# ivargr/kmer_mapper

Measured on AMD Instinct MI355X. Metric: M k-mers mapped/sec (whole node), k=31 150bp reads, higher is better.
Workload: dtype u64

## Files before the change

### kmer_mapper_amd/csrc/kmm.hip

```cpp
#include <hip/hip_runtime.h>

#include <cstdarg>
#include <cstdint>
#include <cstdio>
#include <cstdlib>
#include <chrono>
#include <cstring>
#include <memory>
#include <mutex>
#include <string>
#include <thread>
#include <utility>
#include <vector>

#include "kmm.h"
#include "kmm_radix_plan.hpp"

namespace {

thread_local std::string g_err;

int fail(int code, const char *fmt, ...)
{
    char buf[1024];
// ... 287 lines not shown
    int64_t bgzf_carry_len = 0;
    BgzfStaged bgzf_pre;
    bool bgzf_pre_valid = false;
    const uint8_t *bgzf_pre_from = nullptr, *bgzf_hint_ptr = nullptr;
    int64_t bgzf_pre_n = 0, bgzf_hint_n = 0;
    int bgzf_pre_buf = 0;
    int64_t bgzf_prestaged_calls = 0;
    int64_t bgzf_head_skip = 0;
    int64_t bgzf_tail_stop = -1;
    int64_t bgzf_calls = 0, bgzf_members = 0;
    DevBuf gz_comp, gz_raw, gz_carry, gz_window, gz_tabs, gz_meta, gz_res, gz_win, gz_gmaps, gz_gwin, gz_err;
    std::vector<DevBuf> gz_arena;
    kmm_gunzip::StreamState gz_state;
    int64_t gz_carry_len = 0;
    double gz_ratio = 4.0;
    int64_t gzip_calls = 0, gzip_members = 0, gzip_chunks = 0, gzip_false_starts = 0, gzip_continuations = 0, gzip_inflated = 0;
    int dbg_gzip_chunk_kb = 0;
    DevBuf bam_tiles[2], bam_bad, bam_base, bam_ctl, bam_out;
    int32_t bam_n_ref = -1;
    uint32_t bam_excl = 0;
    int64_t bam_calls = 0, bam_records = 0, bam_excluded = 0, bam_header_bytes = 0, bam_false_starts = 0, bam_continuations = 0;
    int64_t dbg_bgzf_call_cap_kb = 0;
    int64_t flat_uniform_batches = 0;
    DevBuf sam_tiles, sam_base, sam_ctl;
    int64_t sam_calls = 0, sam_records = 0, sam_excluded = 0, sam_header_lines = 0;
    int dbg_bgzf_slot_kb = 0;
    int64_t dbg_rx_buf_limit = 0;
    int dbg_rec_copy_stream = 0;
    int dbg_rec_skip = 0;
    int min_base_quality = 0;
    int64_t dbg_rec_piece_kb = 0;
    bool rx_filter = true;
    bool rx_filter_slots = true;
    uint32_t dbg_p2f_cap = P2F_SLOTS;
    bool rx_packed = true;
    bool ecnt_dirty = false;
    bool rx_unchecked = false;
    DevBuf rx_buf1, rx_buf2, rx_meta, rx_probe;
    int sticky_rc = KMM_OK;
    std::string sticky_msg;
    uint64_t map_calls = 0;
    uint64_t n_radix_batches = 0, n_direct_batches = 0;
    ncclComm_t comm = nullptr;
    int comm_rank = -1, comm_size = 0;
    int comm_slices = 8;
    int64_t comm_sliced_reduces = 0;
    Stream comm_stream;
    std::vector<Event> comm_events;
    std::vector<uint64_t> flush_cuts;
    bool timing = false;
    std::vector<TimedEvent> ev_used;
    std::vector<TimedEvent> ev_free;
    double ms_total[KMM_N_KERNELS] = {0};
    int64_t launches[KMM_N_KERNELS] = {0};
};

namespace {

IndexView view_of(const kmm_index *ix)
{
    IndexView v;
    v.buckets = ix->buckets;
    v.entries = ix->entries;
    v.occ = ix->use_occ ? ix->occ : nullptr;
    v.occ_shift = ix->occ_shift;
    v.bloom_words = ix->bloom_words;
// ... 3135 lines not shown
{
    if (!ix || !name)
        return fail(KMM_ERR_INVALID_ARG, "NULL argument");
    HIPCHK(hipSetDevice(ix->device));
    if (strncmp(name, "debug_records_", 14) != 0)
        HIPCHK(hipStreamSynchronize(ix->stream));
    if (!strcmp(name, "path")) {
        if (value < 0 || value > 2)
            return fail(KMM_ERR_INVALID_ARG, "path must be 0 (auto), 1 (direct) or 2 (radix)");
        if (value == 2 && !ix->rx_ok)
            return fail(KMM_ERR_INVALID_ARG, "the radix path is not available for this index (modulo %llu: needs modulo < 2^31 "
                        "and slices whose entries fit LDS)", (unsigned long long)ix->modulo);
        ix->path = (int)value;
    } else if (!strcmp(name, "part_shift")) {
        const int rc = rx_reconfigure(ix, (int)value, -1, true);
        if (rc == RX_REFUSED)
            return fail(KMM_ERR_INVALID_ARG, "part_shift %lld: needs 0 <= shift <= 13, at most 512 x 512 fine partitions "
                        "and 2^shift small enough for the quotient of a 64-bit k-mer by the modulo to fit beside "
                        "the hash bits", (long long)value);
        KMMCHK(rc);
    } else if (!strcmp(name, "radix_packed_tiles")) {
        ix->rx_packed = value != 0;
    } else if (!strcmp(name, "radix_filter")) {
        ix->rx_filter = value != 0;
        if (ix->rx_pstart) {
            const int rc = rx_reconfigure(ix, ix->rx_geo.w, -1, false);
            if (rc != RX_REFUSED)
                KMMCHK(rc);
        }
    } else if (!strcmp(name, "radix_filter_slots")) {
        ix->rx_filter_slots = value != 0;
        if (ix->rx_pstart && ix->rx_ok)
            KMMCHK(rx_build_slots(ix));
    } else if (!strcmp(name, "debug_p2f_round_slots")) {
        if (value < 512 || value > P2F_SLOTS || (value & 1))
            return fail(KMM_ERR_INVALID_ARG, "debug_p2f_round_slots must be even and in [512, %d]", P2F_SLOTS);
        ix->dbg_p2f_cap = (uint32_t)value;
    } else if (!strcmp(name, "fine_bits")) {
        const int rc = value < 0 || value > 9 ? RX_REFUSED : rx_reconfigure(ix, ix->rx_geo.w, (int)value, true);
        if (rc == RX_REFUSED)
            return fail(KMM_ERR_INVALID_ARG, "fine_bits %lld: both fan-outs must stay within 512", (long long)value);
        KMMCHK(rc);
    } else if (!strcmp(name, "radix_min_units")) {
        ix->rx_min_units = value;
    } else if (!strcmp(name, "radix_sub_batch_kmers")) {
        if (value < 4 * RX_B || value > ((int64_t)1 << 32) - 2 * RX_B)
            return fail(KMM_ERR_INVALID_ARG, "radix_sub_batch_kmers outside [%d, 2^32 - %d]", 4 * RX_B, 2 * RX_B);
        ix->rx_sub_cap = value;
        ix->rx_sub_cap_eff = 0;
    } else if (!strcmp(name, "comm_overlap_slices")) {
        if (value < 1 || value > 64)
            return fail(KMM_ERR_INVALID_ARG, "comm_overlap_slices outside [1, 64]");
        ix->comm_slices = (int)value;
        ix->flush_cuts.clear();
    } else if (!strcmp(name, "radix_sorted_flush")) {
        ix->rx_flush_sorted = value != 0;
    } else if (!strcmp(name, "radix_grid_per_cu")) {
        if (value < 1 || value > 2)
            return fail(KMM_ERR_INVALID_ARG, "radix_grid_per_cu must be 1 or 2");
        ix->rx_grid_per_cu = (int)value;
    } else if (!strcmp(name, "count_kmers")) {
        if (value && !ix->rx_ok)
            return fail(KMM_ERR_INVALID_ARG, "count_kmers needs the radix path, which is not available for this index");
        KMMCHK(rx_flush(ix));
        HIPCHK(hipStreamSynchronize(ix->stream));
        if (value && !ix->rx_ecnt_acc) {
// ... 171 lines not shown
        } else {
            const size_t ld = (size_t)ix->dbg_F1 + 1;
            std::vector<uint16_t> r((size_t)ix->dbg_NB * ld);
            HIPCHK(hipMemcpy(r.data(), ix->dbg_start1, r.size() * 2, hipMemcpyDeviceToHost));
            for (size_t b = 0; b < ix->dbg_NB; ++b)
                sum += r[b * ld + ld - 1];
        }
        *value = (int64_t)sum;
    }
    else if (!strcmp(name, "radix_sorted_flush"))
        *value = (ix->rx_flush_sorted && ix->rx_norder) ? 1 : 0;
    else if (!strcmp(name, "radix_available"))
        *value = ix->rx_ok ? 1 : 0;
    else if (!strcmp(name, "radix_batches"))
        *value = (int64_t)ix->n_radix_batches;
    else if (!strcmp(name, "direct_batches"))
        *value = (int64_t)ix->n_direct_batches;
    else if (!strcmp(name, "radix_unavailable_reason"))
        *value = ix->rx_ok ? 0 : ix->rx_why_not;
    else if (!strcmp(name, "direct_view_resident"))
        *value = ix->buckets ? 1 : 0;
    else if (!strcmp(name, "direct_view_bytes"))
        *value = (int64_t)ix->direct_bytes;
    else if (!strcmp(name, "radix_view_bytes"))
        *value = ix->rx_pstart ? (int64_t)rx_view_bytes(ix->modulo, ix->rx_S, ix->rx_norder != nullptr) : 0;
    else if (!strcmp(name, "radix_filter"))
        *value = (ix->rx_ok && rx_filter_active(ix)) ? 1 : 0;
    else if (!strcmp(name, "radix_p3_keys_in_lds"))
        *value = ix->rx_ok ? rx_p3_shape(rx_p3_variant(ix)).keys_in_lds : 0;
    else if (!strcmp(name, "radix_filter_buckets_per_bit"))
        *value = (ix->rx_ok && rx_filter_active(ix)) ? (1 << ix->rx_geo.occ_shift) : 0;
    else if (!strcmp(name, "radix_filter_slots"))
        *value = (ix->rx_ok && rx_slots_active(ix)) ? 1 : 0;
    else if (!strcmp(name, "radix_filter_bits_per_partition"))
        *value = !(ix->rx_ok && rx_filter_active(ix)) ? 0
                 : rx_slots_active(ix)                ? (int64_t)P2F_SLOT_WORDS * 32
                                                      : (int64_t)1 << (ix->rx_geo.w + ix->rx_geo.f2 - ix->rx_geo.occ_shift);
    else if (!strcmp(name, "debug_p2f_round_slots"))
        *value = ix->dbg_p2f_cap;
    else if (!strcmp(name, "radix_packed_tiles"))
        *value = ix->rx_packed ? 1 : 0;
    else if (!strcmp(name, "n_fine_per_coarse"))
        *value = ix->rx_ok ? ix->rx_geo.F2 : 0;
    else if (!strcmp(name, "count_kmers"))
        *value = ix->rx_ecnt_acc ? 1 : 0;
    else if (!strcmp(name, "n_coarse_partitions"))
        *value = ix->rx_ok ? ix->rx_geo.F1 : 0;
    else if (!strcmp(name, "radix_p2_kmers") || !strcmp(name, "radix_p3_kmers") || !strcmp(name, "radix_p2_dropped") ||
             !strcmp(name, "radix_p2_multi_round_items") || !strcmp(name, "quality_masked_bases") || !strncmp(name, "stats_slot_", 11)) {
        HIPCHK(hipSetDevice(ix->device));
        KMMCHK(drain(ix));
        std::vector<unsigned long long> st(KMM_STAT_BYTES / 8);
        HIPCHK(hipMemcpy(st.data(), ix->stats, KMM_STAT_BYTES, hipMemcpyDeviceToHost));
        const int slot = name[0] == 's' ? atoi(name + 11) : name[0] == 'q' ? KMM_STAT_QUAL_MASKED
                                                          : !strcmp(name, "radix_p2_dropped") ? KMM_STAT_RX_DROPPED
                                                          : !strcmp(name, "radix_p2_multi_round_items") ? KMM_STAT_RX_MULTI
                                                          : name[7] == '2' ? 2 : 3;
        if (slot < 0 || slot >= KMM_STAT_STRIDE)
            return fail(KMM_ERR_INVALID_ARG, "unknown parameter '%s'", name);
        unsigned long long t = 0;
        for (int i = 0; i < KMM_STAT_SHARDS; ++i)
            t += st[(size_t)i * KMM_STAT_STRIDE + slot];
        *value = (int64_t)t;
    }
    else if (!strcmp(name, "grid_per_cu"))
        *value = ix->grid_per_cu;
    else if (!strcmp(name, "dynamic_schedule"))
        *value = ix->dynamic_schedule ? 1 : 0;
    else if (!strcmp(name, "occupancy_filter"))
        *value = (ix->use_occ && ix->occ) ? 1 : 0;
    else if (!strcmp(name, "bloom_filter_bytes"))
        *value = (ix->use_occ && ix->occ) ? (int64_t)ix->bloom_words * 4 : 0;
    else if (!strcmp(name, "occupancy_bits_per_bucket"))
        *value = (ix->use_occ && ix->occ && !ix->bloom_words) ? (1 << ix->occ_shift) : 0;
    else if (!strcmp(name, "wide_buckets"))
        *value = ix->wide ? 1 : 0;
    else if (!strcmp(name, "n_partitions"))
        *value = ix->rx_ok ? ix->rx_geo.PF : 0;
    else
        return fail(KMM_ERR_INVALID_ARG, "unknown parameter '%s'", name);
    return KMM_OK;
}

}
```

### kmer_mapper_amd/csrc/kmm_probe.hpp

```cpp
#pragma once

typedef uint32_t u32x4 __attribute__((ext_vector_type(4)));

struct IndexView {
    const uint4 *buckets;
    const uint4 *entries;
    const uint32_t *occ;
    int occ_shift;
    uint32_t bloom_words;
    int wide;
    uint32_t *counts;
    unsigned long long *stats;
    uint64_t modulo;
    uint64_t magic;
};

struct ReadsView {
    const uint8_t *bases;
    int64_t total;
    const int64_t *offsets;
    int64_t n_reads;
    const uint32_t *start_bits;
    int64_t n_start_words;
    uint64_t read_len;
// ... 43 lines not shown
    return q;
}


__device__ __forceinline__ uint32_t wave_scan_incl(uint32_t v)
{
    v += (uint32_t)__builtin_amdgcn_update_dpp(0, (int)v, 0x111, 0xF, 0xF, false);
    v += (uint32_t)__builtin_amdgcn_update_dpp(0, (int)v, 0x112, 0xF, 0xF, false);
    v += (uint32_t)__builtin_amdgcn_update_dpp(0, (int)v, 0x114, 0xF, 0xF, false);
    v += (uint32_t)__builtin_amdgcn_update_dpp(0, (int)v, 0x118, 0xF, 0xF, false);
    v += (uint32_t)__builtin_amdgcn_update_dpp(0, (int)v, 0x142, 0xA, 0xF, false);
    v += (uint32_t)__builtin_amdgcn_update_dpp(0, (int)v, 0x143, 0xC, 0xF, false);
    return v;
}

__device__ __forceinline__ uint64_t revcomp(uint64_t x, int k)
{
    x = ~x;
    x = ((x >> 2) & 0x3333333333333333ull) | ((x & 0x3333333333333333ull) << 2);
    x = ((x >> 4) & 0x0F0F0F0F0F0F0F0Full) | ((x & 0x0F0F0F0F0F0F0F0Full) << 4);
    x = ((x >> 8) & 0x00FF00FF00FF00FFull) | ((x & 0x00FF00FF00FF00FFull) << 8);
    x = ((x >> 16) & 0x0000FFFF0000FFFFull) | ((x & 0x0000FFFF0000FFFFull) << 16);
    x = (x >> 32) | (x << 32);
    return x >> (64 - 2 * k);
}

__device__ __forceinline__ uint32_t kmer_fp16(uint64_t q)
{
    return (uint32_t)((q * 0x9E3779B97F4A7C15ull) >> 48);
}

constexpr int KMM_STAT_SHARDS = 256;
constexpr int KMM_STAT_STRIDE = 32;
constexpr int KMM_STAT_RX_P1 = 16, KMM_STAT_RX_DROPPED = 17, KMM_STAT_RX_MULTI = 18, KMM_STAT_QUAL_MASKED = 19;
constexpr int AGG_LOG_SLOTS = 11;
constexpr int AGG_SLOTS = 1 << AGG_LOG_SLOTS;
constexpr uint32_t AGG_EMPTY = 0xFFFFFFFFu;

struct NodeAgg {
    uint32_t key[AGG_SLOTS];
    uint32_t val[AGG_SLOTS];
    uint32_t st[2];
};

__device__ __forceinline__ void agg_init(NodeAgg &agg)
{
    for (int i = threadIdx.x; i < AGG_SLOTS; i += blockDim.x) {
        agg.key[i] = AGG_EMPTY;
        agg.val[i] = 0;
    }
    if (threadIdx.x < 2)
        agg.st[threadIdx.x] = 0;
}

__device__ __forceinline__ void agg_add_n(const IndexView &iv, NodeAgg &agg, uint32_t node, uint32_t inc)
{
    const uint32_t slot = (node * 2654435761u) >> (32 - AGG_LOG_SLOTS);
    const uint32_t prev = atomicCAS(&agg.key[slot], AGG_EMPTY, node);
    if (prev == AGG_EMPTY || prev == node)
        atomicAdd(&agg.val[slot], inc);
    else
        atomicAdd(&iv.counts[node], inc);
}

__device__ __forceinline__ void agg_add(const IndexView &iv, NodeAgg &agg, uint32_t node, uint32_t &hits)
{
    ++hits;
// ... 208 lines not shown
```

### kmer_mapper_amd/csrc/kmm_radix.hpp

```cpp
#pragma once
#include <type_traits>
#include "kmm_radix_plan.hpp"

constexpr int RX_NT = 512;
constexpr int RX_KPT = RX_B / RX_NT;
#ifndef RX_LPR2V
#define RX_LPR2V 16
#endif
constexpr int RX_LPR = RX_LPR2V;
constexpr int RX_NG = RX_NT / RX_LPR;
#ifndef RX_RB1
#define RX_RB1 4
#endif
#ifndef RX_RB2
#define RX_RB2 8
#endif
constexpr int RX_SUBCAP = 1024;
#ifndef RX_SUBCAP3V
#define RX_SUBCAP3V 3072
#endif
constexpr int RX_SUBCAP3 = RX_SUBCAP3V;
#ifndef RX_LPR3
#define RX_LPR3 16
#endif
// ... 1356 lines not shown
        put_table(rd, item_lo(0), item_lo(0) + item_n(0), 0);
        if (n_it > 1u)
            rd = load_desc(s_b0[1]);
        __syncthreads();
        cover = t_vs[P2F_NT];
        vm0 = fill(std::false_type(), b0, item_lo(0), item_n(0), item_lo(0), cover, x0, 0);
        __syncthreads();
        if (cover < item_lo(0) + item_n(0))
            more_rounds(0, x0, vm0);
        if (tid < RX_B / 32)
            t_sbits[0][tid] = 0u;
        if (tid == 0)
            t_empty[0] = 0u;
        if (n_it > 1u) {
            put_table(rd, item_lo(1), item_lo(1) + item_n(1), 1);
            if (n_it > 2u)
                rd = load_desc(s_b0[2]);
        }
        __syncthreads();
        for (uint32_t j = 0; j < n_it; j += 2u) {
            process(j, x0, vm0, x1, vm1);
            if (j + 1u < n_it)
                process(j + 1u, x1, vm1, x0, vm0);
        }
    }
    }
#ifndef RX_PT_P1
    RX_PT_END(iv, 10);
#endif
    rx_stat_add(iv, 2, gathered);
    rx_stat_add(iv, KMM_STAT_RX_DROPPED, dropped);
}

template <int WMAX, int ECAP, int WPS, typename DirT, int SUBCAP = RX_SUBCAP3, bool P16 = false>
__global__ void __launch_bounds__(RX_NT, WPS) k_rx_p3(IndexView iv, RxView rx, int max_freq)
{
    static_assert(!P16 || sizeof(DirT) == 2, "the 16-bit directory is copied as it is");
    __shared__ __attribute__((aligned(4))) DirT sdir[WMAX + 2];
    __shared__ uint64_t skeys[ECAP];
    __shared__ uint32_t scnt[ECAP];
    __shared__ uint32_t sub_list[SUBCAP];
    __shared__ uint32_t s_wb[RX_MAXF + 1], s_wave8[2][RX_NT / 64];
    __shared__ uint32_t s_idx;
    const int tid = threadIdx.x, grp = tid / RX_LPR_P3, lg = tid % RX_LPR_P3;
    const uint32_t n_rows = rx.ctrl[1], F1 = rx.F1, F2 = rx.F2;
    const uint32_t W = 1u << rx.w;
    const uint64_t M = iv.modulo;
    for (uint32_t i = tid; i <= F1; i += RX_NT)
        s_wb[i] = rx.work_base[i];
    const uint32_t gs = (F2 + 7u) / 8u, limit = n_rows * gs;
    unsigned long long *counters = rx.queue + 128;
    const uint32_t home = rx_xcc_id();
    uint32_t hits = 0, probed = 0, scan_flip = 0;
    __syncthreads();
    struct Slice {
        uint32_t valid, g, e0, ne, it0, n_it, over, tot, fmax;
        uint64_t h0;
    };
    auto describe = [&](uint32_t sub, uint32_t idx) {
        Slice d;
        d.valid = 0; d.g = 0; d.e0 = 0; d.ne = 0; d.it0 = 0; d.n_it = 0; d.h0 = 0; d.over = 0; d.tot = 0; d.fmax = 0xFFFFu;
        if (idx >= limit)
            return d;
        const uint32_t row = idx / gs, g = sub * gs + idx % gs;
        uint32_t c_lo = 0, c_hi = F1;
        while (c_hi - c_lo > 1) {
            const uint32_t mid = (c_lo + c_hi) >> 1;
            if (s_wb[mid] <= row)
                c_lo = mid;
            else
                c_hi = mid;
        }
        const uint32_t c = c_lo;
        const uint32_t f2c = rx.PF - c * F2 < F2 ? rx.PF - c * F2 : F2;
        if (g >= f2c)
            return d;
        const uint32_t chunk = row - s_wb[c];
        d.valid = 1;
        d.g = g;
        d.h0 = (uint64_t)(c * F2 + g) << rx.w;
        uint32_t e1;
        if (P16) {
            d.e0 = rx.slice_e0[c * F2 + g];
            e1 = rx.slice_e0[c * F2 + g + 1u];
            d.fmax = rx.slice_fmax ? (uint32_t)rx.slice_fmax[c * F2 + g] : 0xFFFFu;
        } else {
// ... 65 lines not shown
        const uint16_t *rfp = rx.start2T + (size_t)g * rx.max_items + it0;
        const uint16_t *rtp = rfp + rx.max_items;
#pragma unroll
        for (int j = 0; j < RX_IC / RX_NT; ++j) {
            const uint32_t i = tid + j * RX_NT;
            rf[j] = i < n_it ? rfp[i] : 0u;
            rt[j] = i < n_it ? rtp[i] : 0u;
        }
        if (P16) {
            uint32_t *sd32 = reinterpret_cast<uint32_t *>(sdir);
#pragma unroll
            for (int j = 0; j < WMAX / 2 / RX_NT; ++j) {
                const uint32_t i = tid + j * RX_NT;
                if (i < W / 2u)
                    sd32[i] = dv[j];
            }
            if (W < 2u && tid == 0)
                sdir[0] = (DirT)dv[0];
            if (tid == 0)
                sdir[W] = (DirT)sl.tot;
        } else {
#pragma unroll
            for (int j = 0; j <= WMAX / RX_NT; ++j) {
                const uint32_t i = tid + j * RX_NT;
                if (i <= W)
                    sdir[i] = (DirT)(dv[j] - e0);
            }
        }
#pragma unroll
        for (int j = 0; j < ECAP / RX_NT; ++j) {
            const uint32_t i = tid + j * RX_NT;
            if (i < ne) {
                skeys[i] = kv[j];
                scnt[i] = (int)fv[j] <= max_freq ? 0u : RX_FILTERED;
            }
        }
        }
        RX_PT(1);
        if (tid == 0)
            s_idx = nxt;
        __syncthreads();
        const uint32_t idx_n = s_idx;
        if (tid == 0 && idx_n < limit)
            nxt = rx_pop(counters, sub, limit);
        const Slice sl_n = describe(sub, idx_n);
        auto probe_bucket_hbm = [&](uint64_t q, uint32_t st, uint32_t cn) {
            for (uint32_t j = 0; j < cn; ++j) {
                const size_t e = (size_t)e0 + st + j;
                if (rx.pkeys[e] == q && (int)rx.pfreq[e] <= max_freq) {
                    atomicAdd(&rx.ecnt[e], 1u);
                    ++hits;
                }
            }
        };
        if (sl.valid) {
        {
            constexpr int NR = RX_IC / RX_NT;
            uint32_t len[NR], np[NR], np_sum = 0, src[NR];
#pragma unroll
            for (int j = 0; j < NR; ++j) {
                len[j] = rt[j] - rf[j];
                src[j] = (uint32_t)(tid + j * RX_NT) * (uint32_t)RX_B + rf[j];
                np[j] = (len[j] + (uint32_t)RX_LPR_P3 - 1u) / (uint32_t)RX_LPR_P3;
                np_sum += np[j];
            }
            const char *wbase = reinterpret_cast<const char *>(rx.buf2 + (size_t)__builtin_amdgcn_readfirstlane((int)it0) * RX_B);
// ... 35 lines not shown
                            const size_t far = ((size_t)it0 * RX_B + (e[u] >> 5) + (uint32_t)lg) % ((size_t)rx.NB * RX_B);
                            const uint64_t z = RX_LOAD3(rx.buf1 + far);
                            asm volatile("" ::"v"(z));
                        }
#endif
                    }
                    return act;
                };
                auto probe = [&](auto over_tag, const uint64_t (&x)[RX_U], uint32_t actm) {
                    constexpr bool OVER = decltype(over_tag)::value;
#pragma unroll
                    for (int g0 = 0; g0 < RX_U; g0 += RX_G3) {
                        uint32_t st[RX_G3], cn[RX_G3];
#pragma unroll
                        for (int i = 0; i < RX_G3; ++i) {
                            const uint32_t hb = (uint32_t)x[g0 + i] & (W - 1u);
                            st[i] = sdir[hb];
                            cn[i] = sdir[hb + 1];
                        }
                        uint32_t mx = 0;
#pragma unroll
                        for (int i = 0; i < RX_G3; ++i) {
                            const bool act = (actm >> (g0 + i)) & 1u;
                            probed += act ? 1u : 0u;
                            cn[i] = act ? cn[i] - st[i] : 0u;
                            if constexpr (OVER) {
                                if (cn[i] && st[i] + cn[i] > ne) {
                                    probe_bucket_hbm(x[g0 + i], st[i], cn[i]);
                                    cn[i] = 0;
                                }
                            }
                            mx = cn[i] > mx ? cn[i] : mx;
                        }
                        for (uint32_t j = 0; j < mx; ++j) {
                            uint64_t key[RX_G3];
#pragma unroll
                            for (int i = 0; i < RX_G3; ++i)
                                key[i] = skeys[j < cn[i] ? st[i] + j : 0u];
#pragma unroll
                            for (int i = 0; i < RX_G3; ++i)
                                if (j < cn[i] && key[i] == x[g0 + i])
                                    atomicAdd(&scnt[st[i] + j], 1u);
                        }
                    }
                };
                auto stream = [&](auto over_tag) {
                    for (uint32_t bi = 0; bi < n_bat; ++bi) {
                        uint64_t x[RX_U];
                        const uint32_t m = request(grp + bi * STEP, x);
                        probe(over_tag, x, m);
                    }
                };
                if (sl.over)
                    stream(std::true_type());
                else
                    stream(std::false_type());
                __syncthreads();
                RX_PT(3);
            }
        }
        for (uint32_t i = tid; i < ne; i += RX_NT) {
            const uint32_t cn = scnt[i];
            if (cn - 1u < RX_FILTERED - 1u) {
                atomicAdd(&rx.ecnt[(size_t)e0 + i], cn);
                hits += cn;
            }
        }
        }
        RX_PT(4);
        __syncthreads();
        if (idx_n >= limit)
            break;
        sl = sl_n;
    }
    }
    RX_PT_END(iv, 4);
    rx_stat_add(iv, 1, hits);
    rx_stat_add(iv, 3, probed);
}

__global__ void __launch_bounds__(256) k_rx_flush(IndexView iv, uint32_t *__restrict__ ecnt,
                                                  const uint32_t *__restrict__ pnodes, uint64_t n,
                                                  uint32_t *__restrict__ ecnt_acc)
{
    __shared__ NodeAgg agg;
    agg_init(agg);
    __syncthreads();
    auto one = [&](uint64_t e, uint32_t cn, uint32_t node) {
        if (cn) {
            if (ecnt_acc)
                ecnt_acc[e] += cn;
            agg_add_n(iv, agg, node, cn);
        }
    };
    const uint64_t n4 = n / 4, gid = (uint64_t)blockIdx.x * 256 + threadIdx.x, stride = (uint64_t)gridDim.x * 256;
    uint4 *c4 = reinterpret_cast<uint4 *>(ecnt);
    const uint4 *n4p = reinterpret_cast<const uint4 *>(pnodes);
    for (uint64_t i = gid; i < n4; i += stride) {
        const uint4 c = c4[i];
        const uint4 nd = n4p[i];
        if (c.x | c.y | c.z | c.w) {
            c4[i] = make_uint4(0u, 0u, 0u, 0u);
            one(4 * i, c.x, nd.x);
            one(4 * i + 1, c.y, nd.y);
            one(4 * i + 2, c.z, nd.z);
            one(4 * i + 3, c.w, nd.w);
        }
    }
    for (uint64_t e = n4 * 4 + gid; e < n; e += stride) {
        const uint32_t cn = ecnt[e];
        if (cn) {
// ... 228 lines not shown
```

### kmer_mapper_amd/csrc/kmm_radix_host.hpp

```cpp
#pragma once

int rx_check_conservation(kmm_index *ix)
{
    if (!ix->rx_unchecked)
        return KMM_OK;
    ix->rx_unchecked = false;
    static thread_local std::vector<unsigned long long> st;
    st.resize(KMM_STAT_BYTES / 8);
    HIPCHK(hipMemcpy(st.data(), ix->stats, KMM_STAT_BYTES, hipMemcpyDeviceToHost));
    unsigned long long p1 = 0, p2 = 0, p3 = 0, dropped = 0;
    for (int i = 0; i < KMM_STAT_SHARDS; ++i) {
        const unsigned long long *sh = st.data() + (size_t)i * KMM_STAT_STRIDE;
        p1 += sh[KMM_STAT_RX_P1];
        p2 += sh[2];
        p3 += sh[3];
        dropped += sh[KMM_STAT_RX_DROPPED];
    }
    if (p1 == p2 && p2 == p3 + dropped)
        return KMM_OK;
    const int rc = fail(KMM_ERR_INTERNAL, "radix path self-check failed: pass 1 emitted %llu k-mers, pass 2 gathered %llu, "
                        "pass 3 probed %llu (+ %llu dropped as absent) since the counters were last reset: the node counts "
                        "are invalid until kmm_reset_counts [latest map call #%llu on this handle]",
                        p1, p2, p3, dropped, (unsigned long long)ix->map_calls);
    ix->sticky_rc = rc;
    ix->sticky_msg = g_err;
    return rc;
}

bool rx_filter_active(const kmm_index *ix)
{
    const RxGeometry &g = ix->rx_geo;
    return ix->rx_filter && ix->rx_occ && g.w + g.f2 - g.occ_shift >= 5 && g.occ_shift <= 2;
}

bool rx_slots_active(const kmm_index *ix)
{
    return rx_filter_active(ix) && ix->rx_geo.slot_filter && ix->rx_filter_slots && ix->rx_slots;
}

bool use_radix(const kmm_index *ix, int64_t units)
{
    if (!ix->rx_ok || ix->path == 1)
        return false;
    return ix->path == 2 || ix->rx_ecnt_acc || units >= ix->rx_min_units;
}

RxP3Variant rx_p3_variant(const kmm_index *ix)
{
    return rx_choose_p3(ix->rx_geo.w, ix->rx_fits_small, ix->rx_fits_mid, ix->rx_pstart16 != nullptr, ix->rx_max_slice,
                        ix->rx_no_mid);
}

RxView rx_view_of(const kmm_index *ix, const RxScratch &sc, uint32_t NB)
{
    const RxGeometry &g = ix->rx_geo;
    RxView rx;
    memset(&rx, 0, sizeof rx);
    rx.pstart = ix->rx_pstart; rx.pkeys = ix->rx_pkeys; rx.pfreq = ix->rx_pfreq; rx.ecnt = ix->rx_ecnt;
    rx.pstart16 = ix->rx_pstart16; rx.slice_e0 = ix->rx_slice_e0; rx.slice_fmax = ix->rx_slice_fmax;
    rx.occ = ix->rx_occ;
    rx.slots = rx_slots_active(ix) ? (const uint32_t *)ix->rx_slots : nullptr;
    rx.p2f_cap = ix->dbg_p2f_cap;
    rx.occ_shift = rx_filter_active(ix) ? g.occ_shift : 3;
    rx.p2f_k = NB / 2048u < 4u ? 4u : (NB / 2048u > (uint32_t)P2F_KMAX ? (uint32_t)P2F_KMAX : NB / 2048u);
    rx.w = g.w; rx.f2 = g.f2; rx.PF = g.PF; rx.F1 = g.F1; rx.F2 = g.F2;
    rx.NB = NB; rx.max_items = (uint32_t)sc.max_items;
    uint8_t *m = (uint8_t *)ix->rx_meta.p;
    rx.start1 = (uint16_t *)(m + sc.start1); rx.P1T = (uint32_t *)(m + sc.P1T); rx.S1T = (uint16_t *)(m + sc.S1T);
    rx.csum = (uint32_t *)(m + sc.csum); rx.T1 = (uint32_t *)(m + sc.T1); rx.item_base = (uint32_t *)(m + sc.item_base);
    rx.work_base = (uint32_t *)(m + sc.work_base); rx.item_desc = (uint2 *)(m + sc.item_desc);
    rx.start2 = (uint16_t *)(m + sc.start2); rx.start2T = (uint16_t *)(m + sc.start2T);
    rx.ctrl = (uint32_t *)(m + sc.ctrl);
    rx.queue = (unsigned long long *)(m + sc.queue);
    rx.buf1 = (uint64_t *)ix->rx_buf1.p;
    rx.buf2 = (uint64_t *)ix->rx_buf2.p;
#if RX_PROBE_ANY
    rx.probe = (uint64_t *)ix->rx_probe.p;
#endif
    return rx;
}

template <int MODE>
int rx_launch_p1(kmm_index *ix, const ReadsView &rv, const uint64_t *src_kmers, int64_t n_kmers, const IndexView &iv,
// ... 12 lines not shown
        if (rv.codes2) {
            if (also_rc)
                go(k_rx_p1<MODE, true, true>);
            else
                go(k_rx_p1<MODE, false, true>);
            return KMM_OK;
        }
    }
    if (also_rc)
        go(k_rx_p1<MODE, true>);
    else
        go(k_rx_p1<MODE, false>);
    return KMM_OK;
}

void rx_launch_p2(kmm_index *ix, const IndexView &iv, const RxView &rx)
{
    if (!ix->rx_filter) {
        hipLaunchKernelGGL(k_rx_p2, dim3(ix->n_cu * ix->rx_grid_per_cu), dim3(RX_NT), 0, ix->stream, iv, rx);
        return;
    }
    const bool flt = rx_filter_active(ix), small = rx.F2 <= 128;
    auto kern = rx.slots ? (small ? k_rx_p2f<P2F_SLOT, true> : k_rx_p2f<P2F_SLOT, false>)
                : flt    ? (small ? k_rx_p2f<P2F_BITMAP, true> : k_rx_p2f<P2F_BITMAP, false>)
                         : (small ? k_rx_p2f<P2F_NONE, true> : k_rx_p2f<P2F_NONE, false>);
    hipLaunchKernelGGL(kern, dim3(ix->n_cu), dim3(P2F_NT), 0, ix->stream, iv, rx);
}

void rx_launch_p3(kmm_index *ix, const IndexView &iv, const RxView &rx, int max_freq)
{
    const RxP3Variant v = rx_p3_variant(ix);
    const dim3 grid(ix->n_cu * (rx_p3_shape(v).wg_per_cu > 1 ? ix->rx_grid_per_cu : 1));
    auto go = [&](auto kern) { hipLaunchKernelGGL(kern, grid, dim3(RX_NT), 0, ix->stream, iv, rx, max_freq); };
    switch (v) {
    case RxP3Variant::W12_DIR16:       go(k_rx_p3<RX_WMAX, RX_ECAP, 4, uint16_t, RX_SUBCAP3, true>); break;
    case RxP3Variant::W12:             go(k_rx_p3<RX_WMAX, RX_ECAP, 4, uint32_t>); break;
    case RxP3Variant::W13_SMALL_DIR16: go(k_rx_p3<RX_WMAX_BIG, RX_ECAP, 4, uint16_t, RX_SUBCAP3, true>); break;
    case RxP3Variant::W13_SMALL:       go(k_rx_p3<RX_WMAX_BIG, RX_ECAP, 4, uint16_t>); break;
    case RxP3Variant::W13_MID_DIR16:   go(k_rx_p3<RX_WMAX_BIG, RX_ECAP_MID, 4, uint16_t, 1024, true>); break;
    case RxP3Variant::W13_MID:         go(k_rx_p3<RX_WMAX_BIG, RX_ECAP_MID, 4, uint16_t, 1024>); break;
    case RxP3Variant::W13_BIG:         go(k_rx_p3<RX_WMAX_BIG, RX_ECAP_BIG, 2, uint32_t>); break;
    }
}

template <int MODE>
int launch_rx(kmm_index *ix, const ReadsView &rv, const uint64_t *kmers_in, int64_t n_in, int k, int max_freq,
              int also_rc)
{
    const IndexView iv = view_of(ix);
    const int64_t units = MODE == MODE_KMERS ? n_in : rv.total;
    const int64_t n_src_total = MODE == MODE_PACKED ? (rv.n_reads + 2 * (int64_t)rv.pk_rpt - 1) / (2 * (int64_t)rv.pk_rpt)
                                                    : (units + RX_B - 1) / RX_B;
    const uint32_t X = also_rc ? 2u : 1u;
    const uint32_t F1 = ix->rx_geo.F1, F2 = ix->rx_geo.F2;
    RxSplit split;
    static const bool verbose = getenv("KMM_VERBOSE") != nullptr;
    const auto t_0 = std::chrono::steady_clock::now();
    if (ix->rx_sub_cap_eff > 0 && ++ix->rx_sub_cap_eff_age >= RX_SUB_CAP_AGE)
        ix->rx_sub_cap_eff = 0;
    int64_t cap = ix->rx_sub_cap_eff > 0 && ix->rx_sub_cap_eff < ix->rx_sub_cap ? ix->rx_sub_cap_eff : ix->rx_sub_cap;
    for (;;) {
        split = rx_split(n_src_total, X, cap);
        const RxScratch sm = rx_scratch((uint32_t)(split.max_src * X), F1, F2);
        int rc = ix->dbg_rx_buf_limit && sm.buf1_bytes > (size_t)ix->dbg_rx_buf_limit ? (int)KMM_ERR_NOMEM
                                                                                      : ensure(ix->rx_meta, sm.meta_bytes);
        if (rc == KMM_OK)
            rc = ensure(ix->rx_buf1, sm.buf1_bytes);
        if (rc == KMM_OK)
// ... 121 lines not shown
    ix->rx_max_slice = (uint32_t)mx[0];
    const unsigned long long odd = ix->rx_geo.PF / 1000 > 1 ? ix->rx_geo.PF / 1000 : 1;
    ix->rx_fits_small = mx[1] <= odd;
    ix->rx_fits_mid = mx[2] <= odd;
    static_cast<RxDir16 &>(*ix) = RxDir16();
    if (ix->rx_max_slice <= 65535u && !getenv("KMM_RX_NO_P16")) {
        const size_t n16 = ((size_t)ix->rx_geo.PF << ix->rx_geo.w) + 8;
        if (hipMalloc(ix->rx_pstart16.put(), n16 * 2) == hipSuccess &&
            hipMalloc(ix->rx_slice_e0.put(), ((size_t)ix->rx_geo.PF + 2) * 4) == hipSuccess &&
            hipMalloc(ix->rx_slice_fmax.put(), ((size_t)ix->rx_geo.PF + 2) * 2) == hipSuccess) {
            hipLaunchKernelGGL(k_rx_pstart16, dim3(grid_for(ix, (int64_t)((n16 + 255) / 256), 16)), dim3(256), 0, ix->stream,
                               ix->rx_pstart, ix->modulo, ix->rx_geo.w, ix->rx_geo.PF, ix->rx_pstart16, ix->rx_slice_e0);
            HIPCHK(hipGetLastError());
            hipLaunchKernelGGL(k_rx_slice_fmax, dim3(grid_for(ix, (int64_t)((ix->rx_geo.PF + 3) / 4), 16)), dim3(256), 0, ix->stream,
                               ix->rx_slice_e0, ix->rx_pfreq, ix->rx_geo.PF, ix->rx_slice_fmax);
            HIPCHK(hipGetLastError());
            HIPCHK(hipStreamSynchronize(ix->stream));
        } else {
            (void)hipGetLastError();
            static_cast<RxDir16 &>(*ix) = RxDir16();
        }
    }
    return rx_build_slots(ix);
}

int rx_build(kmm_index *ix, const int32_t *h2i, const int32_t *nk, const uint64_t *kmers, const int32_t *nodes,
             const uint16_t *freqs)
{
    const uint64_t M = ix->modulo;
    if (const char *env = getenv("KMM_RX_FILTER"))
        ix->rx_filter = atoi(env) != 0;
    if (const char *env = getenv("KMM_RX_FILTER_SLOTS"))
        ix->rx_filter_slots = atoi(env) != 0;
    ix->rx_why_not = 1;
    if (M >= (1ull << 31))
        return KMM_OK;
    DevBuf sizes;
    std::vector<DevBuf> scratch(2 * SCAN_MAX_LEVELS);
    int rc = KMM_OK;
    hipError_t e = hipSuccess;
    bool overlap = false;
    do {
        if ((rc = ensure(sizes, (size_t)(M + 1) * 4))) break;
        if ((e = hipMalloc(ix->rx_pstart.put(), (size_t)(M + 1) * RxViewBytes::pstart))) break;
        hipLaunchKernelGGL(k_rx_bucket_sizes, dim3(grid_for(ix, (int64_t)((M + 256) / 256), 16)), dim3(256), 0,
                           ix->stream, h2i, nk, M, ix->n_entries, (uint32_t *)sizes.p);
        unsigned long long sum64 = 0;
        if ((e = hipMemsetAsync(ix->queue, 0, sizeof(unsigned long long), ix->stream))) break;
        hipLaunchKernelGGL(k_sum_u32, dim3(grid_for(ix, (int64_t)((M + 256) / 256), 8)), dim3(256), 0, ix->stream,
                           (const uint32_t *)sizes.p, M + 1, ix->queue);
        if ((e = hipMemcpyAsync(&sum64, ix->queue, 8, hipMemcpyDeviceToHost, ix->stream))) break;
        if ((e = hipStreamSynchronize(ix->stream))) break;
        if (sum64 > (unsigned long long)ix->n_entries) {
            overlap = true;
            break;
        }
        if ((rc = scan_exclusive((const uint32_t *)sizes.p, ix->rx_pstart, M + 1, scratch, 0, ix->stream))) break;
        uint32_t total = 0;
        if ((e = hipMemcpyAsync(&total, ix->rx_pstart + M, 4, hipMemcpyDeviceToHost, ix->stream))) break;
        if ((e = hipStreamSynchronize(ix->stream))) break;
        ix->rx_S = total;
        {
            const size_t occ_words = (size_t)((M + 31) / 32) + ((size_t)1 << (P2F_LOGBITS + 2 - 5));
            if (hipMalloc(ix->rx_occ.put(), occ_words * 4) == hipSuccess) {
                if ((e = hipMemsetAsync(ix->rx_occ, 0, occ_words * 4, ix->stream))) break;
                hipLaunchKernelGGL(k_rx_build_occ, dim3(grid_for(ix, (int64_t)((M / 32 + 256) / 256), 16)), dim3(256), 0, ix->stream,
// ... 101 lines not shown
```

### kmer_mapper_amd/csrc/kmm_radix_plan.hpp

```cpp
#pragma once
#include <cstddef>
#include <cstdint>
#include <optional>

constexpr int RX_B = 8192;
constexpr int RX_MAXF = 512;
#ifndef RX_CHV
#define RX_CHV 256
#endif
constexpr int RX_CH = RX_CHV;
constexpr int RX_IC = 1024;
constexpr int RX_ECAP = 4096;
constexpr int RX_ECAP_BIG = 8192;
constexpr int RX_ECAP_MID = 4608;
constexpr int P2F_KMAX = 64;
constexpr int P2F_LOGBITS = 19;
constexpr int P2F_SLOT_WORDS = 3 << (P2F_LOGBITS - 6);
constexpr int P2F_SLOTS = 5888;

constexpr uint32_t rx_filter_slot(uint32_t b, uint64_t quot)
{
    const uint32_t v = ((uint32_t)quot ^ (uint32_t)(quot >> 24) ^ (uint32_t)(quot >> 48)) + (b << 23);
    const uint32_t h16 = ((v & 0xFFFFFFu) * 0x9E3779u) >> 16;
    return 3u * (b >> 1) + ((h16 * 3u) >> 16);
}

struct RxGeometry {
    int w = 12, f2 = 0;
    int occ_shift = 0;
    bool slot_filter = false;
    uint32_t PF = 1, F1 = 1, F2 = 1;
};

inline std::optional<RxGeometry> rx_geometry(uint64_t modulo, uint64_t S, bool filter, int w, int maxf = RX_MAXF, int f2_force = -1)
{
    if (w < 0 || w > 13 || modulo == 0 || modulo >= (1ull << 31))
        return std::nullopt;
    const uint64_t PF = (modulo + (1ull << w) - 1) >> w;
    if (PF > (uint64_t)maxf * maxf)
        return std::nullopt;
    int lg = 0;
    while ((1ull << lg) < PF)
        ++lg;
    int f2 = (lg + 1) / 2;
    bool for_filter = false;
    if (filter && w + f2 > P2F_LOGBITS) {
        const double load = S ? (double)S / (double)modulo : 0.5;
        for (int gs = 0; gs <= 2 && !for_filter; ++gs) {
            const int fb = P2F_LOGBITS + gs - w;
            if (fb < 0 || load * (double)(1 << gs) > 0.75)
                continue;
            if (((PF + (1ull << fb) - 1) >> fb) <= (uint64_t)RX_MAXF && fb <= 9) {
                f2 = fb;
                for_filter = true;
            }
        }
    }
// ... 89 lines not shown
struct RxSplit {
    int64_t n_sub, max_src;
};

inline RxSplit rx_split(int64_t n_src_total, uint32_t X, int64_t cap)
{
    const int64_t cap_src = (cap / RX_B) / X > 0 ? (cap / RX_B) / X : 1;
    RxSplit s;
    s.n_sub = (n_src_total + cap_src - 1) / cap_src;
    s.max_src = s.n_sub ? (n_src_total + s.n_sub - 1) / s.n_sub : cap_src;
    return s;
}

inline int64_t rx_next_smaller_cap(int64_t n_src_total, uint32_t X, int64_t n_sub)
{
    const int64_t next_src = (n_src_total + n_sub) / (n_sub + 1);
    const int64_t cap = next_src * RX_B * X;
    return cap < RX_SUB_CAP_FLOOR ? RX_SUB_CAP_FLOOR : cap;
}

enum class RxP3Variant {
    W12_DIR16,
    W12,
    W13_SMALL_DIR16,
    W13_SMALL,
    W13_MID_DIR16,
    W13_MID,
    W13_BIG,
};
struct RxP3Shape {
    int keys_in_lds;
    int wg_per_cu;
    bool dir16;
};
constexpr RxP3Shape RX_P3_SHAPES[] = {
    {RX_ECAP, 2, true}, {RX_ECAP, 2, false},
    {RX_ECAP, 2, true}, {RX_ECAP, 2, false},
    {RX_ECAP_MID, 2, true}, {RX_ECAP_MID, 2, false},
    {RX_ECAP_BIG, 1, false},
};
constexpr const RxP3Shape &rx_p3_shape(RxP3Variant v) { return RX_P3_SHAPES[(int)v]; }

inline RxP3Variant rx_choose_p3(int w, bool fits_small, bool fits_mid, bool p16, uint32_t max_slice, bool no_mid)
{
    if (w <= 12)
        return p16 ? RxP3Variant::W12_DIR16 : RxP3Variant::W12;
    const bool lds16 = p16 || max_slice <= 65535u;
    if (fits_small && lds16)
        return p16 ? RxP3Variant::W13_SMALL_DIR16 : RxP3Variant::W13_SMALL;
    if (fits_mid && lds16 && !no_mid)
        return p16 ? RxP3Variant::W13_MID_DIR16 : RxP3Variant::W13_MID;
    return RxP3Variant::W13_BIG;
}

struct RxViewBytes {
    enum : size_t { pstart = 4, pkeys = 8, pkeys_raw = 8, pfreq = 2, pnodes = 4, porig = 4, ecnt = 4, norder = 4, nnode = 4 };
};
constexpr size_t rx_view_bytes(uint64_t modulo, uint64_t S, bool node_order)
{
    return (size_t)(modulo + 1) * RxViewBytes::pstart +
           (size_t)(S ? S : 1) * (RxViewBytes::pkeys + RxViewBytes::pkeys_raw + RxViewBytes::pfreq + RxViewBytes::pnodes +
                                  RxViewBytes::porig + RxViewBytes::ecnt + (node_order ? RxViewBytes::norder + RxViewBytes::nnode : 0));
}

inline int64_t rx_min_units(uint64_t modulo, uint64_t S)
{
    const double bytes = (double)modulo * 4.0 + (double)S * 14.0;
    const double fixed = 50e-6 + bytes / 2.6e12;
    const double per_kmer_radix = 6.5e-12 * (1.0 + bytes / 40e9);
    const double per_kmer_direct = 1.0 / (bytes < 1e9 ? 60e9 : 38e9);
    const int64_t units = (int64_t)(1.25 * fixed / (per_kmer_direct - per_kmer_radix));
    return units < ((int64_t)1 << 22) ? (int64_t)1 << 22 : units;
}
```

Measured before the change: 169,900.

## Add 8-bit fingerprint prefilter to radix phase-3 LDS key probing

Phase 3 of the radix path now also stores an 8-bit hash fingerprint for each staged index key in shared memory. Each query compares its fingerprint against the first five entries of its bucket with SWAR byte matching, and reads the 64-bit key from LDS only on a fingerprint hit. Entries past the fifth are still scanned linearly. This is meant to cut LDS key reads and compare work, at the cost of extra shared memory, hashing during staging, and more complex control flow; it applies only to the W12_DIR16 variant and is on by default.

Result: faster. 172,500 (median of 6 runs) (+1.6%).

```diff
diff --git a/kmer_mapper_amd/csrc/kmm.hip b/kmer_mapper_amd/csrc/kmm.hip
--- a/kmer_mapper_amd/csrc/kmm.hip
+++ b/kmer_mapper_amd/csrc/kmm.hip
@@ -343,6 +343,7 @@
     int64_t dbg_rec_piece_kb = 0;
     bool rx_filter = true;
     bool rx_filter_slots = true;
+    bool rx_p3_fp = true;
     uint32_t dbg_p2f_cap = P2F_SLOTS;
     bool rx_packed = true;
     bool ecnt_dirty = false;
@@ -3544,6 +3545,8 @@
         ix->rx_filter_slots = value != 0;
         if (ix->rx_pstart && ix->rx_ok)
             KMMCHK(rx_build_slots(ix));
+    } else if (!strcmp(name, "radix_p3_fingerprints")) {
+        ix->rx_p3_fp = value != 0;
     } else if (!strcmp(name, "debug_p2f_round_slots")) {
         if (value < 512 || value > P2F_SLOTS || (value & 1))
             return fail(KMM_ERR_INVALID_ARG, "debug_p2f_round_slots must be even and in [512, %d]", P2F_SLOTS);
@@ -3781,6 +3784,8 @@
         *value = (ix->rx_ok && rx_filter_active(ix)) ? (1 << ix->rx_geo.occ_shift) : 0;
     else if (!strcmp(name, "radix_filter_slots"))
         *value = (ix->rx_ok && rx_slots_active(ix)) ? 1 : 0;
+    else if (!strcmp(name, "radix_p3_fingerprints"))
+        *value = (ix->rx_ok && rx_p3_fp_active(ix)) ? 1 : 0;
     else if (!strcmp(name, "radix_filter_bits_per_partition"))
         *value = !(ix->rx_ok && rx_filter_active(ix)) ? 0
                  : rx_slots_active(ix)                ? (int64_t)P2F_SLOT_WORDS * 32
@@ -3796,12 +3801,14 @@
     else if (!strcmp(name, "n_coarse_partitions"))
         *value = ix->rx_ok ? ix->rx_geo.F1 : 0;
     else if (!strcmp(name, "radix_p2_kmers") || !strcmp(name, "radix_p3_kmers") || !strcmp(name, "radix_p2_dropped") ||
-             !strcmp(name, "radix_p2_multi_round_items") || !strcmp(name, "quality_masked_bases") || !strncmp(name, "stats_slot_", 11)) {
+             !strcmp(name, "radix_p2_multi_round_items") || !strcmp(name, "quality_masked_bases") ||
+             !strcmp(name, "debug_p3_key_reads") || !strncmp(name, "stats_slot_", 11)) {
         HIPCHK(hipSetDevice(ix->device));
         KMMCHK(drain(ix));
         std::vector<unsigned long long> st(KMM_STAT_BYTES / 8);
         HIPCHK(hipMemcpy(st.data(), ix->stats, KMM_STAT_BYTES, hipMemcpyDeviceToHost));
         const int slot = name[0] == 's' ? atoi(name + 11) : name[0] == 'q' ? KMM_STAT_QUAL_MASKED
+                                                          : name[0] == 'd' ? KMM_STAT_RX_P3_KEYS
                                                           : !strcmp(name, "radix_p2_dropped") ? KMM_STAT_RX_DROPPED
                                                           : !strcmp(name, "radix_p2_multi_round_items") ? KMM_STAT_RX_MULTI
                                                           : name[7] == '2' ? 2 : 3;
diff --git a/kmer_mapper_amd/csrc/kmm_probe.hpp b/kmer_mapper_amd/csrc/kmm_probe.hpp
--- a/kmer_mapper_amd/csrc/kmm_probe.hpp
+++ b/kmer_mapper_amd/csrc/kmm_probe.hpp
@@ -99,7 +99,7 @@
 
 constexpr int KMM_STAT_SHARDS = 256;
 constexpr int KMM_STAT_STRIDE = 32;
-constexpr int KMM_STAT_RX_P1 = 16, KMM_STAT_RX_DROPPED = 17, KMM_STAT_RX_MULTI = 18, KMM_STAT_QUAL_MASKED = 19;
+constexpr int KMM_STAT_RX_P1 = 16, KMM_STAT_RX_DROPPED = 17, KMM_STAT_RX_MULTI = 18, KMM_STAT_QUAL_MASKED = 19, KMM_STAT_RX_P3_KEYS = 20;
 constexpr int AGG_LOG_SLOTS = 11;
 constexpr int AGG_SLOTS = 1 << AGG_LOG_SLOTS;
 constexpr uint32_t AGG_EMPTY = 0xFFFFFFFFu;
diff --git a/kmer_mapper_amd/csrc/kmm_radix.hpp b/kmer_mapper_amd/csrc/kmm_radix.hpp
--- a/kmer_mapper_amd/csrc/kmm_radix.hpp
+++ b/kmer_mapper_amd/csrc/kmm_radix.hpp
@@ -1412,10 +1412,16 @@
     rx_stat_add(iv, KMM_STAT_RX_DROPPED, dropped);
 }
 
-template <int WMAX, int ECAP, int WPS, typename DirT, int SUBCAP = RX_SUBCAP3, bool P16 = false>
+#ifdef RX_P3_FP_STATS
+#define RX_P3_KEY_READ(cond) key_reads += (cond) ? 1u : 0u
+#else
+#define RX_P3_KEY_READ(cond)
+#endif
+template <int WMAX, int ECAP, int WPS, typename DirT, int SUBCAP = RX_SUBCAP3, bool P16 = false, bool FP = false>
 __global__ void __launch_bounds__(RX_NT, WPS) k_rx_p3(IndexView iv, RxView rx, int max_freq)
 {
     static_assert(!P16 || sizeof(DirT) == 2, "the 16-bit directory is copied as it is");
+    __shared__ uint32_t sfp[FP ? (ECAP + 8) / 4 : 1];
     __shared__ __attribute__((aligned(4))) DirT sdir[WMAX + 2];
     __shared__ uint64_t skeys[ECAP];
     __shared__ uint32_t scnt[ECAP];
@@ -1432,6 +1438,10 @@
     unsigned long long *counters = rx.queue + 128;
     const uint32_t home = rx_xcc_id();
     uint32_t hits = 0, probed = 0, scan_flip = 0;
+#ifdef RX_P3_FP_STATS
+    uint32_t key_reads = 0;
+#endif
+    const int sh = rx.w + rx.f2;
     __syncthreads();
     struct Slice {
         uint32_t valid, g, e0, ne, it0, n_it, over, tot, fmax;
@@ -1563,6 +1573,8 @@
             const uint32_t i = tid + j * RX_NT;
             if (i < ne) {
                 skeys[i] = kv[j];
+                if constexpr (FP)
+                    reinterpret_cast<uint8_t *>(sfp)[i] = (uint8_t)rx_p3_fp(kv[j] >> sh);
                 scnt[i] = (int)fv[j] <= max_freq ? 0u : RX_FILTERED;
             }
         }
@@ -1664,11 +1676,57 @@
                             }
                             mx = cn[i] > mx ? cn[i] : mx;
                         }
-                        for (uint32_t j = 0; j < mx; ++j) {
+                        if constexpr (FP) {
+                            uint32_t f0[RX_G3], f1[RX_G3], fp4[RX_G3], cm[RX_G3], any = 0;
+#pragma unroll
+                            for (int i = 0; i < RX_G3; ++i) {
+                                const uint32_t wi = (OVER && !cn[i] ? 0u : st[i]) >> 2;
+                                f0[i] = sfp[wi];
+                                f1[i] = sfp[wi + 1u];
+                            }
+#pragma unroll
+                            for (int i = 0; i < RX_G3; ++i) {
+                                fp4[i] = rx_p3_fp4(x[g0 + i] >> sh);
+                                const uint32_t lo = __builtin_amdgcn_alignbit(f1[i], f0[i], 8u * st[i]);
+                                cm[i] = rx_p3_match4(lo, fp4[i], cn[i]);
+                                any |= cm[i];
+                            }
+                            while (any) {
+                                uint64_t key[RX_G3];
+                                uint32_t e8[RX_G3];
+#pragma unroll
+                                for (int i = 0; i < RX_G3; ++i) {
+                                    e8[i] = cm[i] ? 8u * st[i] + (uint32_t)__builtin_ctz(cm[i]) : 0u;
+                                    key[i] = *reinterpret_cast<const uint64_t *>(reinterpret_cast<const char *>(skeys) + e8[i]);
+                                    RX_P3_KEY_READ(cm[i] != 0u);
+                                }
+                                any = 0;
+#pragma unroll
+                                for (int i = 0; i < RX_G3; ++i) {
+                                    if (cm[i] && key[i] == x[g0 + i])
+                                        atomicAdd(reinterpret_cast<uint32_t *>(reinterpret_cast<char *>(scnt) + (e8[i] >> 1)), 1u);
+                                    cm[i] &= cm[i] - 1u;
+                                    any |= cm[i];
+                                }
+                            }
+                            if (mx >= (uint32_t)RX_P3_FP_ENTRIES) {
+#pragma unroll
+                                for (int i = 0; i < RX_G3; ++i) {
+                                    if (rx_p3_match_entry4(f1[i] >> (8u * (st[i] & 3u)), fp4[i], cn[i])) {
+                                        RX_P3_KEY_READ(true);
+                                        if (skeys[st[i] + 4u] == x[g0 + i])
+                                            atomicAdd(&scnt[st[i] + 4u], 1u);
+                                    }
+                                }
+                            }
+                        }
+                        for (uint32_t j = FP ? RX_P3_FP_ENTRIES : 0; j < mx; ++j) {
                             uint64_t key[RX_G3];
 #pragma unroll
-                            for (int i = 0; i < RX_G3; ++i)
+                            for (int i = 0; i < RX_G3; ++i) {
                                 key[i] = skeys[j < cn[i] ? st[i] + j : 0u];
+                                RX_P3_KEY_READ(j < cn[i]);
+                            }
 #pragma unroll
                             for (int i = 0; i < RX_G3; ++i)
                                 if (j < cn[i] && key[i] == x[g0 + i])
@@ -1709,6 +1767,9 @@
     RX_PT_END(iv, 4);
     rx_stat_add(iv, 1, hits);
     rx_stat_add(iv, 3, probed);
+#ifdef RX_P3_FP_STATS
+    rx_stat_add(iv, KMM_STAT_RX_P3_KEYS, key_reads);
+#endif
 }
 
 __global__ void __launch_bounds__(256) k_rx_flush(IndexView iv, uint32_t *__restrict__ ecnt,
diff --git a/kmer_mapper_amd/csrc/kmm_radix_host.hpp b/kmer_mapper_amd/csrc/kmm_radix_host.hpp
--- a/kmer_mapper_amd/csrc/kmm_radix_host.hpp
+++ b/kmer_mapper_amd/csrc/kmm_radix_host.hpp
@@ -49,6 +49,11 @@
 {
     return rx_choose_p3(ix->rx_geo.w, ix->rx_fits_small, ix->rx_fits_mid, ix->rx_pstart16 != nullptr, ix->rx_max_slice,
                         ix->rx_no_mid);
+}
+
+bool rx_p3_fp_active(const kmm_index *ix)
+{
+    return ix->rx_p3_fp && rx_p3_shape(rx_p3_variant(ix)).fingerprints;
 }
 
 RxView rx_view_of(const kmm_index *ix, const RxScratch &sc, uint32_t NB)
@@ -127,8 +132,15 @@
     const RxP3Variant v = rx_p3_variant(ix);
     const dim3 grid(ix->n_cu * (rx_p3_shape(v).wg_per_cu > 1 ? ix->rx_grid_per_cu : 1));
     auto go = [&](auto kern) { hipLaunchKernelGGL(kern, grid, dim3(RX_NT), 0, ix->stream, iv, rx, max_freq); };
+    static_assert(rx_p3_shape(RxP3Variant::W12_DIR16).fingerprints && rx_p3_fp_shapes() == 1,
+                  "RX_P3_SHAPES promises the fingerprint form exactly where an instantiation is named below");
     switch (v) {
-    case RxP3Variant::W12_DIR16:       go(k_rx_p3<RX_WMAX, RX_ECAP, 4, uint16_t, RX_SUBCAP3, true>); break;
+    case RxP3Variant::W12_DIR16:
+        if (rx_p3_fp_active(ix))
+            go(k_rx_p3<RX_WMAX, RX_ECAP, 4, uint16_t, RX_SUBCAP3, true, true>);
+        else
+            go(k_rx_p3<RX_WMAX, RX_ECAP, 4, uint16_t, RX_SUBCAP3, true>);
+        break;
     case RxP3Variant::W12:             go(k_rx_p3<RX_WMAX, RX_ECAP, 4, uint32_t>); break;
     case RxP3Variant::W13_SMALL_DIR16: go(k_rx_p3<RX_WMAX_BIG, RX_ECAP, 4, uint16_t, RX_SUBCAP3, true>); break;
     case RxP3Variant::W13_SMALL:       go(k_rx_p3<RX_WMAX_BIG, RX_ECAP, 4, uint16_t>); break;
@@ -316,6 +328,8 @@
         ix->rx_filter = atoi(env) != 0;
     if (const char *env = getenv("KMM_RX_FILTER_SLOTS"))
         ix->rx_filter_slots = atoi(env) != 0;
+    if (const char *env = getenv("KMM_RX_P3_FP"))
+        ix->rx_p3_fp = atoi(env) != 0;
     ix->rx_why_not = 1;
     if (M >= (1ull << 31))
         return KMM_OK;
diff --git a/kmer_mapper_amd/csrc/kmm_radix_plan.hpp b/kmer_mapper_amd/csrc/kmm_radix_plan.hpp
--- a/kmer_mapper_amd/csrc/kmm_radix_plan.hpp
+++ b/kmer_mapper_amd/csrc/kmm_radix_plan.hpp
@@ -23,6 +23,48 @@
     const uint32_t v = ((uint32_t)quot ^ (uint32_t)(quot >> 24) ^ (uint32_t)(quot >> 48)) + (b << 23);
     const uint32_t h16 = ((v & 0xFFFFFFu) * 0x9E3779u) >> 16;
     return 3u * (b >> 1) + ((h16 * 3u) >> 16);
+}
+
+#if defined(__HIPCC__)
+#define RX_PLAN_HD __host__ __device__
+#else
+#define RX_PLAN_HD
+#endif
+constexpr int RX_P3_FP_ENTRIES = 5;
+
+RX_PLAN_HD inline uint32_t rx_p3_fp4(uint64_t quot)
+{
+    const uint32_t v = (uint32_t)quot ^ (uint32_t)(quot >> 24) ^ (uint32_t)(quot >> 48);
+#if defined(__HIP_DEVICE_COMPILE__)
+    const uint32_t h = __umul24(v, 0xB5297Bu);
+    return __builtin_amdgcn_perm(h, h, 0x02020202u);
+#else
+    return (((v & 0xFFFFFFu) * 0xB5297Bu >> 16) & 0xFFu) * 0x01010101u;
+#endif
+}
+RX_PLAN_HD inline uint32_t rx_p3_fp(uint64_t quot) { return rx_p3_fp4(quot) & 0xFFu; }
+
+RX_PLAN_HD inline uint32_t rx_p3_match4(uint32_t lo, uint32_t fp4, uint32_t cn)
+{
+    const uint32_t x = lo ^ fp4;
+    const uint32_t z = ((x - 0x01010101u) & ~x & 0x80808080u) >> 7;
+    const uint32_t width = 8u * cn < 31u ? 8u * cn : 31u;
+    return z & ((1u << width) - 1u);
+}
+RX_PLAN_HD inline uint32_t rx_p3_match_entry4(uint32_t hi, uint32_t fp4, uint32_t cn)
+{
+    const uint32_t x = hi ^ fp4;
+    return cn >= (uint32_t)RX_P3_FP_ENTRIES ? ((x - 1u) & ~x & 0x80u) << 24 : 0u;
+}
+RX_PLAN_HD inline uint32_t rx_p3_first_entry(uint32_t m) { return ((uint32_t)__builtin_ctz(m) + 1u) >> 3; }
+
+RX_PLAN_HD inline uint32_t rx_p3_candidates(uint64_t f, uint32_t fp, uint32_t cn)
+{
+    const uint32_t fp4 = fp * 0x01010101u;
+    uint32_t m = rx_p3_match4((uint32_t)f, fp4, cn) | rx_p3_match_entry4((uint32_t)(f >> 32), fp4, cn), out = 0;
+    for (; m; m &= m - 1u)
+        out |= 1u << rx_p3_first_entry(m);
+    return out;
 }
 
 struct RxGeometry {
@@ -178,14 +220,22 @@
     int keys_in_lds;
     int wg_per_cu;
     bool dir16;
+    bool fingerprints = false;
 };
 constexpr RxP3Shape RX_P3_SHAPES[] = {
-    {RX_ECAP, 2, true}, {RX_ECAP, 2, false},
+    {RX_ECAP, 2, true, true}, {RX_ECAP, 2, false},
     {RX_ECAP, 2, true}, {RX_ECAP, 2, false},
     {RX_ECAP_MID, 2, true}, {RX_ECAP_MID, 2, false},
     {RX_ECAP_BIG, 1, false},
 };
 constexpr const RxP3Shape &rx_p3_shape(RxP3Variant v) { return RX_P3_SHAPES[(int)v]; }
+constexpr int rx_p3_fp_shapes()
+{
+    int n = 0;
+    for (const RxP3Shape &s : RX_P3_SHAPES)
+        n += s.fingerprints ? 1 : 0;
+    return n;
+}
 
 inline RxP3Variant rx_choose_p3(int w, bool fits_small, bool fits_mid, bool p16, uint32_t max_slice, bool no_mid)
 {
```
